# lyndonchan/wsss-analysis

Measured on AMD Instinct MI355X. Metric: images/sec CAM+CRF pseudo-labels, VOC2012 321x321, higher is better.
Workload: dtype f16x3; 1 GPU; resnet50 CAM + dense-CRF (M=21, 10 mean-field iters), 321x321, batch 32 images (=64 samples) per GPU, image-sharded; batch_images=32, num_classes=20, parallelism=image-sharded x1, no collective, steps_per_rank=243

## Files before the change

### include/wsscam.h

```cpp
#ifndef WSSCAM_H
#define WSSCAM_H

#include <stddef.h>
#include <stdint.h>

#ifdef __cplusplus
extern "C" {
#endif

#define WSC_VERSION 100

typedef enum wsc_status {
    WSC_OK = 0,
    WSC_ERR_INVALID = -1,
    WSC_ERR_NO_DEVICE = -2,
    WSC_ERR_HIP = -3,
    WSC_ERR_MISSING_KEY = -4,
    WSC_ERR_SHAPE = -5,
    WSC_ERR_NOMEM = -6,
    WSC_ERR_KEY_RANGE = -7,
    WSC_ERR_CAPACITY = -8,
    WSC_ERR_RANGE = -9
} wsc_status;

// ... 163 lines not shown

int wsc_hsn_gradcam_post(wsc_ctx *ctx, const float *cams_nhwc_dev, int B, int h, int w, int C, int S,
                         const float *gate_dev, float *out_dev, int out_channels, int out_first);
int wsc_hsn_voc_background(wsc_ctx *ctx, const float *Hbg_dev, int B, int Cb, int N, float *y_dev, int Ctot);
int wsc_hsn_class_mass(wsc_ctx *ctx, const float *maps_dev, int n_maps, int N, uint32_t *mass_dev);
int wsc_hsn_background(wsc_ctx *ctx, const uint8_t *rgb_dev, int B, int H, int W, int Ho, int Wo, double *bg_dev);
int wsc_cam_adp_modify(wsc_ctx *ctx, const float *cam_dev, int B, int n_sc, int C, int hw, const double *bg_dev, int mode,
                       const int32_t *use_host, int n_use, const int32_t *adipose_host, int n_adip, const int32_t *exc_host,
                       int n_exc, float *out_dev);
int wsc_hsn_cs_gradcam(wsc_ctx *ctx, const float *H_dev, int B, int C_all, int N, const double *bg_dev,
                       const int32_t *src_of_valid_host, int Cv, int bg_ind, int other_ind,
                       const int32_t *exception_inds_host, int n_exc, const int32_t *adipose_src_host, int n_adip,
                       float *cs_dev, float *y_dev, uint32_t *mass_dev);
int wsc_hsn_gather_unary(wsc_ctx *ctx, const float *maps_dev, const int64_t *chan_off_host, int n_chan, int N,
                         float *unary_dev);


int wsc_crf_create(wsc_ctx *ctx, const uint8_t *rgb_dev, int B, int H, int W, float g_sxy,
                   float bi_sxy, float bi_srgb, wsc_crf **out);
void wsc_crf_destroy(wsc_crf *crf);
int wsc_crf_lattice_sizes(wsc_ctx *ctx, const wsc_crf *crf, int32_t *v_gauss_host,
                          int32_t *v_bilat_host);
int wsc_crf_gaussian_on_chip(const wsc_crf *crf, int M);

int wsc_crf_inference(wsc_ctx *ctx, wsc_crf *crf, const float *unary_dev, int M, float g_compat,
                      float bi_compat, int n_iters, float *q_dev, int32_t *argmax_dev);
int wsc_crf_inference_pm(wsc_ctx *ctx, wsc_crf *crf, const float *unary_pm_dev, int M, float g_compat,
                         float bi_compat, int n_iters, float *q_dev, int32_t *argmax_dev);

int wsc_crf_v_create(wsc_ctx *ctx, const uint8_t *const *rgb_dev, const int32_t *hw_host , int B, float g_sxy,
                     float bi_sxy, float bi_srgb, wsc_crf_v **out);
void wsc_crf_v_destroy(wsc_crf_v *crf);
int wsc_crf_v_num_groups(const wsc_crf_v *crf);
int wsc_crf_v_inference(wsc_ctx *ctx, wsc_crf_v *crf, const float *const *unary_dev, const int32_t *M_host, float g_compat,
                        float bi_compat, int n_iters, float *const *q_dev, int32_t *const *argmax_dev);

#ifdef __cplusplus
}
#endif
#endif
```

### wsss-analysis_amd/csrc/crf.hip

```cpp
#include "common.h"

#include <atomic>
#include <cmath>
#include <cstring>
#include <memory>

namespace {

constexpr unsigned long long EMPTY_KEY = 0xFFFFFFFFFFFFFFFFull;
typedef float f32x2_t __attribute__((ext_vector_type(2)));

struct LatticeDev {
    int d = 0;
    int rep = 1;
    int rows = 0;
    int32_t *offset = nullptr;
    float *bary = nullptr;
    float *norm = nullptr;
    int2 *nbr = nullptr;
    int32_t *tslot_start = nullptr;
    int2 *slot_desc = nullptr;
    float *tent_w = nullptr;
    uint8_t *tent_p = nullptr;
    int32_t *row_slot_start = nullptr;
    int n_tiles = 0, n_slots = 0;
    bool sorted_dest = false;
    long long n_pix = 0;
    int M_cur = 0;
// ... 1628 lines not shown
                uint2 en[3];
                f32x4_t in[3];
#pragma unroll
                for (int jj = 0; jj < 3; ++jj) en[jj] = le[min(i + jj, n - 1)];
#pragma unroll
                for (int jj = 0; jj < 3; ++jj) in[jj] = stage[en[jj].x + l];
#pragma unroll
                for (int jj = 0; jj < 3; ++jj) {
                    const float w = i + jj < n ? __uint_as_float(en[jj].y) : 0.f;
                    const f32x2_t w2 = {w, w}, lo = {in[jj][0], in[jj][1]}, hi = {in[jj][2], in[jj][3]};
                    a01 = __builtin_elementwise_fma(w2, lo, a01);
                    a23 = __builtin_elementwise_fma(w2, hi, a23);
                }
            }
            const f32x4_t acc = {a01[0], a01[1], a23[0], a23[1]};
            if (ok) part[(unsigned)d.y * (unsigned)LP + l] = acc;
        }
        __syncthreads();
    }
}

constexpr int REC_LDS_BYTES = 56;
static_assert(TILE_PIX * REC_LDS_BYTES <= (int)(sizeof(uint2) * GATHER_ENT + sizeof(int2) * GATHER_SB), "record stage");
template <bool SLICE, bool SPLAT, bool GF = false, int FG = 0>
__global__ __launch_bounds__(512) __attribute__((amdgpu_waves_per_eu(4))) void update_splat_kernel(UpdateArgs a) {
    constexpr bool DMA = GF || (!SLICE && SPLAT);
    static_assert(!GF || SLICE, "the GF updates slice");
    static_assert(FG == 0 || GF, "the in-kernel Gaussian message belongs to the GF updates");
    extern __shared__ f32x4_t stage[];
    const int LP = a.LP;
    const int gpw = 64 / LP;
    const int lane = threadIdx.x & 63;
    const int g = lane / LP;
    const int l = lane - g * LP;
    const bool act = g < gpw;
    const int seg0 = g * LP;
    const int nb = gridDim.x, bid = blockIdx.x;
    const int xcd = bid & 7, qq = nb >> 3, rr = nb & 7;
    const int lb = (xcd < rr ? xcd * (qq + 1) : rr * (qq + 1) + (xcd - rr) * qq) + (bid >> 3);
    const int k = lb / a.tg.tpi, j = lb - k * a.tg.tpi;
    const TileBox tb = tile_box(a.tg, j);
    const int np = tb.cw * tb.ch;
    const int N = a.tg.H * a.tg.W;
    const int ppt = (int)(blockDim.x >> 6) * gpw;
    const unsigned cw_magic = tile_div_magic(tb.cw);
    const size_t pix0 = (size_t)k * (size_t)N + (size_t)tb.y0 * (size_t)a.tg.W + (size_t)tb.x0;
    const unsigned LP16 = (unsigned)LP * 16u, l16 = (unsigned)l * 16u;
    constexpr unsigned REC_BYTES = GF ? 52u : 80u;
// ... 72 lines not shown
            o23 = f32x2_t{u[2], u[3]};
        } else {
            o01 = f32x2_t{-u[0], -u[1]};
            o23 = f32x2_t{-u[2], -u[3]};
        }
        if (SLICE) {
            if (!GF) {
#pragma unroll
                for (int r = 0; r < 3; ++r) {
                    const f32x2_t w2 = {w9[r], w9[r]}, lo = {g3[r][0], g3[r][1]}, hi = {g3[r][2], g3[r][3]};
                    o01 = __builtin_elementwise_fma(w2, lo, o01);
                    o23 = __builtin_elementwise_fma(w2, hi, o23);
                }
            }
#pragma unroll
            for (int r = 0; r < 6; ++r) {
                const f32x2_t w2 = {w9[3 + r], w9[3 + r]}, lo = {b6[r][0], b6[r][1]}, hi = {b6[r][2], b6[r][3]};
                o01 = __builtin_elementwise_fma(w2, lo, o01);
                o23 = __builtin_elementwise_fma(w2, hi, o23);
            }
        }
    };
    const int t_first = (int)(threadIdx.x >> 6) * gpw;
    constexpr int EN_G = (TILE_PIX * 3 + 255) / 256, EN_B = (TILE_PIX * 6 + 255) / 256;
    SplatRegs<EN_G> rg;
    if (SPLAT && FG == 0) splat_fetch<EN_G>(a.sg, a.sg.shared ? j : lb, (a.sg.shared ? 0ll : (long long)k * N) + tb.ebase, np, rg);
    int4 cnt = make_int4(0, 0, 0, 0);
    int2 ps[FG > 0 ? FG : 1];
    uint4 tn0 = make_uint4(0, 0, 0, 0);
    if (FG > 0) {
        cnt = a.gt_cnt[j];
        const unsigned lpm = (65536u + (unsigned)LP - 1u) / (unsigned)LP;
        const int2 *trow = a.gt_rows + (size_t)j * a.gt_stride;
#pragma unroll
        for (int it = 0; it < (FG > 0 ? FG : 1); ++it) {
            const int i = (int)threadIdx.x + it * GM_THREADS;
            ps[it] = make_int2(0, 0);
            if (i < a.gt_stride * LP) ps[it] = trow[((unsigned)i * lpm) >> 16];
        }
        if ((int)threadIdx.x < a.gt_stride) tn0 = a.gt_nbr[(size_t)j * a.gt_stride + threadIdx.x];
    }
    if (DMA) {
        const int wvu = __builtin_amdgcn_readfirstlane((int)(threadIdx.x >> 6)), nwv = (int)(blockDim.x >> 6);
        const unsigned lp_magic = (65536u + (unsigned)LP - 1u) / (unsigned)LP;
        const int nE = np * LP;
        for (int u0 = wvu * 64; u0 < nE; u0 += nwv * 64) {
            const unsigned u = min((unsigned)(u0 + lane), (unsigned)(nE - 1));
            const unsigned t = (u * lp_magic) >> 16, ll = u - t * (unsigned)LP;
            const unsigned ty = (t * cw_magic) >> 16, tx = t - __umul24(ty, (unsigned)tb.cw);
            const char *src = u_b + (__umul24(__umul24(ty, (unsigned)a.tg.W) + tx, LP16) + ll * 16u);
            __builtin_amdgcn_global_load_lds((const __attribute__((address_space(1))) void *)src,
                                             (__attribute__((address_space(3))) void *)(reinterpret_cast<char *>(stage) + u0 * 16), 16, 0, 0);
        }
        const int nR = SLICE ? np * 14 : 0;
        for (int d0 = wvu * 64; d0 < nR; d0 += nwv * 64) {
            const unsigned d = min((unsigned)(d0 + lane), (unsigned)(nR - 1));
            const unsigned t = (d * 4682u) >> 16;
            const unsigned kk = min(d - t * 14u, 12u);
            const unsigned ty = (t * cw_magic) >> 16, tx = t - __umul24(ty, (unsigned)tb.cw);
            const char *src = rec_b + (__umul24(__umul24(ty, (unsigned)a.tg.W) + tx, REC_BYTES) + kk * 4u);
            __builtin_amdgcn_global_load_lds((const __attribute__((address_space(1))) void *)src,
                                             (__attribute__((address_space(3))) void *)(const_cast<char *>(lrec) + d0 * 4), 4, 0, 0);
        }
        if (FG == 0) {
            asm volatile("s_waitcnt vmcnt(0)" ::: "memory");
            __syncthreads();
        }
    }
    if constexpr (FG > 0) {
        constexpr int NIT = FG, NPI = FG == 4 ? 3 : 4;
        f32x4_t *gl = reinterpret_cast<f32x4_t *>(reinterpret_cast<char *>(stage + TILE_PIX * LP) + SPLAT_TAB_BYTES);
        const int stride = a.gt_stride, tid = (int)threadIdx.x;
        unsigned *lnb = reinterpret_cast<unsigned *>(gl + (size_t)stride * (size_t)LP);
        const f32x4_t zero = {0.f, 0.f, 0.f, 0.f};
        const f32x4_t *partg = reinterpret_cast<const f32x4_t *>(a.part_g_in) + (a.sg.shared ? (size_t)k * a.sg.n_slots * LP : (size_t)0);
        const int nitems_all = stride * LP;
        const unsigned lp_magic = (65536u + (unsigned)LP - 1u) / (unsigned)LP;
        const uint4 *tn = a.gt_nbr + (size_t)j * stride;
        const unsigned gpix0 = (unsigned)tb.y0 * (unsigned)a.tg.W + (unsigned)tb.x0;
        {
            f32x4_t val[NIT];
#pragma unroll
            for (int it = 0; it < NIT; ++it) {
                const int i = tid + it * GM_THREADS;
                const unsigned v = ((unsigned)i * lp_magic) >> 16, ll = (unsigned)i - v * (unsigned)LP;
                val[it] = zero;
                if (ps[it].y > 0) val[it] = partg[(unsigned)ps[it].x * (unsigned)LP + ll];
            }
            if (tid < stride) reinterpret_cast<uint4 *>(lnb)[tid] = tn0;
            for (int v = tid + GM_THREADS; v < stride; v += GM_THREADS) reinterpret_cast<uint4 *>(lnb)[v] = tn[v];
            int maxc = 0;
#pragma unroll
            for (int it = 0; it < NIT; ++it) maxc = max(maxc, ps[it].y);
            constexpr int UN = NIT <= 4 ? 3 : 2;
            if (maxc > 1) {
                f32x4_t more[UN][NIT];
#pragma unroll
                for (int c = 1; c <= UN; ++c)
#pragma unroll
                    for (int it = 0; it < NIT; ++it) {
                        const int i = tid + it * GM_THREADS;
                        const unsigned v = ((unsigned)i * lp_magic) >> 16, ll = (unsigned)i - v * (unsigned)LP;
                        more[c - 1][it] = zero;
                        if (c < ps[it].y) more[c - 1][it] = partg[(unsigned)(ps[it].x + c) * (unsigned)LP + ll];
                    }
#pragma unroll
                for (int c = 1; c <= UN; ++c)
#pragma unroll
                    for (int it = 0; it < NIT; ++it)
                        if (c < ps[it].y) {
#pragma unroll
                            for (int q = 0; q < 4; ++q) val[it][q] += more[c - 1][it][q];
                        }
            }
            for (int c = UN + 1; c < maxc; ++c) {
                f32x4_t more[NIT];
#pragma unroll
                for (int it = 0; it < NIT; ++it) {
                    const int i = tid + it * GM_THREADS;
                    const unsigned v = ((unsigned)i * lp_magic) >> 16, ll = (unsigned)i - v * (unsigned)LP;
                    more[it] = zero;
                    if (c < ps[it].y) more[it] = partg[(unsigned)(ps[it].x + c) * (unsigned)LP + ll];
                }
#pragma unroll
                for (int it = 0; it < NIT; ++it)
                    if (c < ps[it].y) {
#pragma unroll
                        for (int q = 0; q < 4; ++q) val[it][q] += more[it][q];
                    }
            }
#pragma unroll
            for (int it = 0; it < NIT; ++it) {
                const int i = tid + it * GM_THREADS;
                if (i < nitems_all) gl[i] = val[it];
            }
        }
        asm volatile("s_waitcnt vmcnt(0)" ::: "memory");
        uint4 gpx[NPI];
#pragma unroll
        for (int it = 0; it < NPI; ++it) {
            const int i = tid + it * GM_THREADS;
            gpx[it] = make_uint4(0, 0, 0, 0);
            if (i < np * LP) {
                const unsigned t = ((unsigned)i * lp_magic) >> 16;
                const unsigned ty = (t * cw_magic) >> 16, tx = t - ty * (unsigned)tb.cw;
                gpx[it] = a.gt_pix[gpix0 + ty * (unsigned)a.tg.W + tx];
            }
        }
        __syncthreads();
#pragma unroll
        for (int axis = 0; axis < 3; ++axis) {
            const int nitems = (axis == 0 ? cnt.z : (axis == 1 ? cnt.y : cnt.x)) * LP;
            f32x4_t o[NIT];
#pragma unroll
            for (int it = 0; it < NIT; ++it) {
                const int i = tid + it * GM_THREADS;
                o[it] = zero;
                if (i < nitems) {
                    const unsigned v = ((unsigned)i * lp_magic) >> 16, ll = (unsigned)i - v * (unsigned)LP;
                    const unsigned w = lnb[v * 4 + axis];
                    const f32x4_t c = gl[i], x1 = gl[(w & 0xffffu) * (unsigned)LP + ll], x2 = gl[(w >> 16) * (unsigned)LP + ll];
#pragma unroll
                    for (int q = 0; q < 4; ++q) o[it][q] = c[q] + 0.5f * (x1[q] + x2[q]);
                }
            }
            __syncthreads();
#pragma unroll
            for (int it = 0; it < NIT; ++it) {
                const int i = tid + it * GM_THREADS;
                if (i < nitems) gl[i] = o[it];
            }
            __syncthreads();
        }
#pragma unroll
        for (int it = 0; it < NPI; ++it) {
            const int i = tid + it * GM_THREADS;
            if (i < np * LP) {
                const unsigned t = ((unsigned)i * lp_magic) >> 16, ll = (unsigned)i - t * (unsigned)LP;
                const uint4 gp = gpx[it];
                const f32x4_t uu = stage[i];
                f32x2_t o01 = {-uu[0], -uu[1]}, o23 = {-uu[2], -uu[3]};
                const float wr[3] = {__uint_as_float(gp.y) * cag, __uint_as_float(gp.z) * cag, __uint_as_float(gp.w) * cag};
#pragma unroll
                for (int r = 0; r < 3; ++r) {
                    const f32x4_t row = gl[((gp.x >> (10 * r)) & 1023u) * (unsigned)LP + ll];
                    const f32x2_t w2 = {wr[r], wr[r]}, lo = {row[0], row[1]}, hi = {row[2], row[3]};
                    o01 = __builtin_elementwise_fma(w2, lo, o01);
                    o23 = __builtin_elementwise_fma(w2, hi, o23);
                }
                stage[i] = f32x4_t{o01[0], o01[1], o23[0], o23[1]};
            }
        }
        if (SPLAT) splat_fetch<EN_G>(a.sg, a.sg.shared ? j : lb, (a.sg.shared ? 0ll : (long long)k * N) + tb.ebase, np, rg);
        __syncthreads();
    }
    auto emit = [&](int t0) {
        const int t = t0 + g;
        const bool ok = act && t < np;
        const unsigned p = pixel_of(t0);
        float e[4] = {e01[0], e01[1], e23[0], e23[1]};
        float mx = -3.0e38f;
#pragma unroll
        for (int kk = 0; kk < 4; ++kk) {
            e[kk] = (ok && 4 * l + kk < a.M) ? e[kk] : -3.0e38f;
            mx = fmaxf(mx, e[kk]);
        }
        for (int o = 4; o > 0; o >>= 1) {
            const float other = __shfl_down(mx, o, 64);
            if (l + o < LP) mx = fmaxf(mx, other);
        }
        mx = __shfl(mx, seg0, 64);
        float ex[4], sum = 0.f;
        const float mxl = mx * 1.44269504088896341f;
#pragma unroll
        for (int kk = 0; kk < 4; ++kk) {
            ex[kk] = __builtin_amdgcn_exp2f(__builtin_fmaf(e[kk], 1.44269504088896341f, -mxl));
            sum += ex[kk];
// ... 19 lines not shown
                    bi = 4 * l + kk;
                }
            for (int o = 4; o > 0; o >>= 1) {
                const float ov = __shfl_down(bv, o, 64);
                const int oi = __shfl_down(bi, o, 64);
                if (l + o < LP && ov > bv) {
                    bv = ov;
                    bi = oi;
                }
            }
            if (ok && l == 0) a.argmax[pix0 + p] = bi;
        }
    };
    {
        {
            const f32x4_t u0 = load_u(t_first);
            f32x4_t g3[3], b6[6];
            float w9[9];
            if (SLICE) {
                load_rec(t_first, rq);
                issue_rows(rq, g3, b6, w9);
            }
            unn = u0;
            if (t_first + ppt < np) {
                if (SLICE) load_rec(t_first + ppt, rq);
                unn = load_u(t_first + ppt);
            }
            fold(u0, g3, b6, w9, e01, e23);
        }
        for (int t0 = t_first; t0 < np; t0 += ppt) {
            const bool has_next = t0 + ppt < np;
            f32x4_t vgn[3], vbn[6];
            float wrn[9];
            const f32x4_t un1 = unn;
            if (SLICE && has_next) issue_rows(rq, vgn, vbn, wrn);
            if (t0 + 2 * ppt < np) {
                if (SLICE) load_rec(t0 + 2 * ppt, rq);
                unn = load_u(t0 + 2 * ppt);
            }
            emit(t0);
            if (has_next) fold(un1, vgn, vbn, wrn, e01, e23);
        }
    }
    if (SPLAT) {
        uint2 *lent = reinterpret_cast<uint2 *>(stage + TILE_PIX * LP);
        int2 *ldesc = reinterpret_cast<int2 *>(lent + GATHER_ENT);
        if (DMA) __syncthreads();
        splat_commit<EN_G>(a.sg, np, rg, lent, ldesc, LP);
        SplatRegs<EN_B> rb;
        splat_fetch<EN_B>(a.sb, a.sb.shared ? j : lb, (a.sb.shared ? 0ll : (long long)k * N) + tb.ebase, np, rb);
        __syncthreads();
        tile_gather(a.sg, rg.s_beg, rg.s_end, k, stage, lent, ldesc, LP, l, g, gpw, act);
        splat_commit<EN_B>(a.sb, np, rb, lent, ldesc, LP);
        __syncthreads();
        tile_gather(a.sb, rb.s_beg, rb.s_end, k, stage, lent, ldesc, LP, l, g, gpw, act);
    }
}

struct GaussMsgArgs {
    const int4 *gt_cnt;
    const int2 *gt_rows;
    const uint4 *gt_nbr;
    const uint4 *gt_pix;
    const float *part;
    const float *u;
    float *e;
    int gt_stride, n_slots, shared, LP, B;
    float cag;
    TileGeom tg;
// ... 634 lines not shown
    WSC_TRY(tmp.alloc(sizeof(float) * L.rows, &va));
    WSC_TRY(tmp.alloc(sizeof(float) * L.rows, &vb));
    WSC_TRY(tmp.alloc(sizeof(float) * (size_t)(L.n_slots + 1), &vp));
    splat_ones(ctx, L, make_geom(crf->H, crf->W), va, vp);
    float *res = blur_all1(ctx, L, va, vb);
    uint32_t *rec_b = nullptr;
    if (D == 5 && !shared && crf->lat[0].gt_rows && !crf->pix_rec_b) WSC_TRY(own.alloc(sizeof(uint32_t) * 13 * (size_t)npix, &rec_b));
    if (!shared && D == 5) {
        hipLaunchKernelGGL(slice_norm_tile_kernel, dim3((unsigned)L.n_tiles), dim3(256), 0, ctx->stream, L.offset, L.bary, dp1,
                           L.alpha, res, make_geom(crf->H, crf->W), L.norm, rec_b, L.tent_w, L.tent_p);
    } else {
        hipLaunchKernelGGL(slice_norm_kernel, dim3(grid1d(npix)), dim3(256), 0, ctx->stream, L.offset, L.bary, dp1,
                           L.alpha, res, npix, L.norm, rec_b);
        hipLaunchKernelGGL(tile_scale_entries_kernel, dim3((unsigned)L.n_tiles), dim3(256), 0, ctx->stream, L.norm, dp1,
                           make_geom(crf->H, crf->W), L.tent_w, L.tent_p);
    }
    WSC_HIP(hipGetLastError());
    if (rec_b) crf->pix_rec_b = rec_b;
    return WSC_OK;
}

size_t update_splat_lds(int LP) { return sizeof(f32x4_t) * TILE_PIX * LP + sizeof(uint2) * GATHER_ENT + sizeof(int2) * GATHER_SB; }
size_t gauss_msg_lds(int LP, int gt_stride) { return ((size_t)LP * sizeof(f32x4_t) + sizeof(uint4)) * (size_t)gt_stride; }
size_t update_fg_lds(int LP, int gt_stride) { return update_splat_lds(LP) + gauss_msg_lds(LP, gt_stride); }
bool update_gf_ok(const wsc_ctx *ctx, const LatticeDev &G, int LP) {
    if (!ctx->opt[WSC_OPT_CRF_GAUSS_ON_CHIP]) return false;
    if (!G.gt_rows || G.rep < 1 || G.gt_stride <= 0) return false;
    if ((long long)G.gt_stride * LP > 6ll * GM_THREADS || (long long)G.gt_stride * LP >= 8192) return false;
    return gauss_msg_lds(LP, G.gt_stride) <= 64 * 1024;
}
bool update_fg_ok(const wsc_ctx *ctx, const LatticeDev &G, int LP) {
    if (!ctx->opt[WSC_OPT_CRF_MSG_IN_UPDATE] || !update_gf_ok(ctx, G, LP)) return false;
    return update_fg_lds(LP, G.gt_stride) <= 80 * 1024;
}
bool gauss_msg_small(int gt_stride, int LP) { return (long long)gt_stride * LP <= 4ll * GM_THREADS && LP <= 6; }

int launch_gauss_msg(wsc_ctx *ctx, hipStream_t st, const GaussMsgArgs &g, double bytes) {
    WscKernelTimer timer(ctx, WSC_K_GAUSS_MSG, bytes);
    const auto kernel = gauss_msg_small(g.gt_stride, g.LP) ? gauss_msg_kernel<4, 3> : gauss_msg_kernel<6, 4>;
    hipLaunchKernelGGL(kernel, dim3((unsigned)(g.B * g.tg.tpi)), dim3(GM_THREADS), gauss_msg_lds(g.LP, g.gt_stride), st, g);
    WSC_HIP(hipGetLastError());
    return WSC_OK;
}

typedef void (*UpdateKernel)(UpdateArgs);
template <bool SLICE, bool GF, int FG>
UpdateKernel update_kernel(bool splat) { return splat ? update_splat_kernel<SLICE, true, GF, FG> : update_splat_kernel<SLICE, false, GF, FG>; }
struct UpdateVariant { UpdateKernel kernel; int threads; size_t lds; };
UpdateVariant update_variant(bool slice, bool splat, bool gf, bool fg, bool small, int LP, int gt_stride) {
    if (fg) return {small ? update_kernel<true, true, 4>(splat) : update_kernel<true, true, 6>(splat), GM_THREADS, update_fg_lds(LP, gt_stride)};
    if (slice && gf) return {update_kernel<true, true, 0>(splat), 256, update_splat_lds(LP)};
    return {slice ? update_kernel<true, false, 0>(splat) : update_kernel<false, false, 0>(splat), 256, splat ? update_splat_lds(LP) : 0};
}
int update_fg_lds_limit(wsc_ctx *ctx, int LP, int gt_stride) {
    if (update_fg_lds(LP, gt_stride) <= 48 * 1024) return WSC_OK;
    for (const bool small : {true, false})
        for (const bool splat : {true, false}) {
            const UpdateKernel k = update_variant(true, splat, true, true, small, LP, gt_stride).kernel;
            WSC_TRY(wsc_set_max_dynamic_lds(ctx, reinterpret_cast<const void *>(k), 96 * 1024));
        }
    return WSC_OK;
}
int launch_update(wsc_ctx *ctx, const UpdateArgs &a, bool slice, bool splat, bool gf, bool fg = false, double fg_bytes = 0.0) {
    const double npix = (double)a.B * a.tg.H * a.tg.W;
    const double by = npix * (2.0 * a.M * 4 + (slice ? (gf ? 6 * 8 + 1.0 * a.M * 4 : 9 * 8 + 2.0 * a.M * 4) : 0.0) +
                              (splat ? 9 * 8 + 2.0 * a.M * 4 : 0.0));
    WscKernelTimer timer(ctx, WSC_K_SLICE_UPDATE, by + (fg ? fg_bytes : 0.0));
    const UpdateVariant v = update_variant(slice, splat, gf, fg, gauss_msg_small(a.gt_stride, a.LP), a.LP, a.gt_stride);
    hipLaunchKernelGGL(v.kernel, dim3((unsigned)(a.B * a.tg.tpi)), dim3(v.threads), v.lds, ctx->stream, a);
    WSC_HIP(hipGetLastError());
    return WSC_OK;
}

SplatTab splat_tab(const LatticeDev &L, float *part) {
    return SplatTab{L.tslot_start, L.slot_desc, L.tent_w, L.tent_p, part, L.n_slots, L.rep > 1 ? 1 : 0, L.d + 1};
}
UpdateArgs update_args(const wsc_crf *crf, int M, float g_compat, float bi_compat, const float *u, float *partg, float *partb) {
    const LatticeDev &G = crf->lat[0], &Bl = crf->lat[1];
    UpdateArgs a;
    a.pix_rec = crf->pix_rec; a.pix_rec_b = crf->pix_rec_b; a.val_g = nullptr; a.val_b = nullptr;
    a.u = u; a.q = nullptr; a.argmax = nullptr;
    a.alpha_g = G.alpha; a.alpha_b = Bl.alpha; a.compat_g = g_compat; a.compat_b = bi_compat;
    a.M = M; a.LP = (M + 3) / 4; a.B = crf->B; a.tg = make_geom(crf->H, crf->W);
    a.g_pix = (unsigned)G.n_pix; a.g_rows = G.rep > 1 ? (unsigned)G.rows : 0u;
    a.sg = splat_tab(G, partg); a.sb = splat_tab(Bl, partb);
    a.gt_cnt = G.gt_cnt; a.gt_rows = G.gt_rows; a.gt_nbr = G.gt_nbr; a.gt_pix = G.gt_pix; a.gt_stride = G.gt_stride;
    a.part_g_in = nullptr;
    return a;
}
GaussMsgArgs gauss_msg_args(const wsc_crf *crf, int M, float g_compat, const float *part, const float *u, float *e) {
    const LatticeDev &G = crf->lat[0];
// ... 106 lines not shown
}

void wsc_crf_destroy(wsc_crf *crf) {
    if (!crf) return;
    if (crf->used_elsewhere && crf->use_ev) (void)hipStreamWaitEvent(crf->ctx->stream, crf->use_ev, 0);
    if (crf->gauss) crf->gauss->users -= 1;
    crf->blocks.release();
    if (crf->use_ev) (void)hipEventDestroy(crf->use_ev);
    delete crf;
}

int wsc_crf_lattice_sizes(wsc_ctx *ctx, const wsc_crf *crf, int32_t *v_gauss_host, int32_t *v_bilat_host) {
    WSC_CHECK(ctx && crf, WSC_ERR_INVALID, "wsc_crf_lattice_sizes: null argument");
    for (int b = 0; b < crf->B; ++b) {
        if (v_gauss_host) v_gauss_host[b] = crf->lat[0].v_per_image[b];
        if (v_bilat_host) v_bilat_host[b] = crf->lat[1].v_per_image[b];
    }
    return WSC_OK;
}

int wsc_crf_gaussian_on_chip(const wsc_crf *crf, int M) {
    if (!crf || M < 1 || M > 32) return 0;
    return update_gf_ok(crf->ctx, crf->lat[0], (M + 3) / 4) ? 1 : 0;
}

static int crf_inference_impl(wsc_ctx *ctx, wsc_crf *crf, const float *unary_dev, bool pixel_major, int M, float g_compat,
                              float bi_compat, int n_iters, float *q_dev, int32_t *argmax_dev);

int wsc_crf_inference(wsc_ctx *ctx, wsc_crf *crf, const float *unary_dev, int M, float g_compat, float bi_compat,
                      int n_iters, float *q_dev, int32_t *argmax_dev) {
    return crf_inference_impl(ctx, crf, unary_dev, false, M, g_compat, bi_compat, n_iters, q_dev, argmax_dev);
}

int wsc_crf_inference_pm(wsc_ctx *ctx, wsc_crf *crf, const float *unary_pm_dev, int M, float g_compat, float bi_compat,
                         int n_iters, float *q_dev, int32_t *argmax_dev) {
    return crf_inference_impl(ctx, crf, unary_pm_dev, true, M, g_compat, bi_compat, n_iters, q_dev, argmax_dev);
}

static int crf_inference_impl(wsc_ctx *ctx, wsc_crf *crf, const float *unary_dev, bool pixel_major, int M, float g_compat,
                              float bi_compat, int n_iters, float *q_dev, int32_t *argmax_dev) {
    WSC_CHECK(ctx && crf && unary_dev, WSC_ERR_INVALID, "wsc_crf_inference: null argument");
    WSC_CHECK(M >= 1 && M <= 32, WSC_ERR_INVALID, "wsc_crf_inference: M=%d outside [1,32]", M);
    WSC_CHECK(n_iters >= 0, WSC_ERR_INVALID, "wsc_crf_inference: n_iters=%d", n_iters);
    WSC_HIP(hipSetDevice(ctx->device));
    const int B = crf->B, N = crf->N;
    const long long npix = (long long)B * N;
// ... 21 lines not shown
    float *partg = (float *)p; p += pg;
    float *partg2 = (float *)p; p += pg;
    float *partb = (float *)p; p += pb;

    crf->lat[0].M_cur = M;
    crf->lat[1].M_cur = M;
    if (n_iters > 0) WSC_TRY(blur_lds_prepare(ctx, crf->lat[1], M));
    const dim3 tgrid((N + TP - 1) / TP, B);
    if (!pixel_major) {
        WscKernelTimer timer(ctx, WSC_K_CRF_MISC, (double)npix * M * 12);
        hipLaunchKernelGGL(init_q_kernel, tgrid, dim3(TP), 2 * (size_t)M * (TP + 1) * sizeof(float), ctx->stream,
                           unary_dev, M, Mp, N, u, n_iters == 0 ? q : (float *)nullptr);
    } else {
        u = const_cast<float *>(unary_dev);
    }
    const bool lds_blur = Bl.bl_ok && Bl.img_row && ctx->opt[WSC_OPT_CRF_BLUR_ON_CHIP];
    const bool no_fork = lds_blur || ctx->profiling;
    if (!no_fork && !ctx->aux_stream) {
        WSC_HIP(hipStreamCreateWithFlags(&ctx->aux_stream, hipStreamNonBlocking));
        WSC_HIP(hipEventCreateWithFlags(&ctx->fork_ev, hipEventDisableTiming));
        WSC_HIP(hipEventCreateWithFlags(&ctx->aux_done_ev, hipEventDisableTiming));
    }
    const bool gf = update_gf_ok(ctx, G, LP);
    const bool fg = gf && update_fg_ok(ctx, G, LP) && update_fg_lds_limit(ctx, LP, G.gt_stride) == WSC_OK;
    if (n_iters > 0) WSC_TRY(gf ? crf_bilateral_records(crf, ctx->stream) : crf_full_records(crf, ctx->stream));
    UpdateArgs a = update_args(crf, M, g_compat, bi_compat, u, partg, partb);
    const GaussMsgArgs gm = gauss_msg_args(crf, M, g_compat, partg, u, q);
    const double gf_bytes = 2.0 * 3.0 * (double)(G.rows - 1) * G.rep * M * 4 + (double)npix * (3 * 8 + 1.0 * M * 4);
    if (n_iters == 0 && pixel_major) {
        a.q = q;
        WSC_TRY(launch_update(ctx, a, false, false, false));
    }
    for (int it = 0; it <= n_iters && n_iters > 0; ++it) {
        const bool last = it == n_iters;
        const bool labels_only = last && q_dev == nullptr && argmax_dev != nullptr;
        a.q = last && !labels_only ? q : nullptr;
        a.argmax = labels_only ? argmax_dev : nullptr;
        a.u = (gf && !fg && it > 0) ? q : u;
        if (fg) {
            a.part_g_in = (it & 1) ? partg : partg2;
            a.sg.part = (it & 1) ? partg2 : partg;
        }
        WSC_TRY(launch_update(ctx, a, it > 0, !last, gf, fg && it > 0, gf_bytes));
        if (last) break;
        const bool fork = !no_fork;
        hipStream_t main_stream = ctx->stream;
        if (fork) {
// ... 148 lines not shown
```

### wsss-analysis_amd/wsscam/_lib.py

```python
import ctypes
import os
import re
import threading

import numpy as np

_HERE = os.path.dirname(os.path.abspath(__file__))
LIB_PATH = os.path.join(_HERE, "libwsscam.so")
HEADER_PATH = os.path.normpath(os.path.join(_HERE, "..", "..", "include", "wsscam.h"))

WSC_OK = 0
WSC_ERR_INVALID = -1
WSC_ERR_NO_DEVICE = -2
WSC_ERR_HIP = -3
WSC_ERR_MISSING_KEY = -4
WSC_ERR_SHAPE = -5
WSC_ERR_NOMEM = -6
WSC_ERR_KEY_RANGE = -7
WSC_ERR_CAPACITY = -8
WSC_ERR_RANGE = -9

ARCH_RESNET50_CAM = 0
ARCH_VGG16_CAM = 1
ARCH_M7_CAM = 2
# ... 82 lines not shown
    "wsc_unary_from_maps": (_i, [_vp, _vp, _i, _i, _i, _f, _vp]),
    "wsc_cam_unary": (_i, [_vp, _vp, _i, _i, _i, _i, _i, _i, _f, _vp]),
    "wsc_cam_unary_pm": (_i, [_vp, _vp, _i, _i, _i, _i, _i, _i, _f, _vp]),
    "wsc_cam_sum_scales": (_i, [_vp, _vp, _i, _i, ctypes.c_longlong, _vp]),
    "wsc_cam_eval_confusion_nn": (_i, [_vp, _vp, _i, _vp, _vp, _vp, _vp, _vp, _vp, _i, _i, _vp, _vp]),
    "wsc_label_confusion_nn": (_i, [_vp, _vp, _i, _vp, _vp, _vp, _vp, _i, _i, _vp, _vp]),
    "wsc_sem_seg_finish": (_i, [_vp, _vp, _i, _vp, _vp, _vp, _vp, _vp, _vp, _i, _f, _vp]),
    "wsc_bilinear_resize": (_i, [_vp, _vp, _i, _i, _i, _vp, _i, _i]),
    "wsc_msf_input_u8": (_i, [_vp, _vp, _i, _vp, _vp, _i, _vp, _vp, _i, _i, _vp]),
    "wsc_resize_u8": (_i, [_vp, _vp, _i, _vp, _vp, _i, _i, _vp]),
    "wsc_label_unary_from_cam": (_i, [_vp, _vp, _i, _i, _i, _f, _f, _vp, _vp]),
    "wsc_ir_label_combine": (_i, [_vp, _vp, _vp, _vp, _i, _i, _i, _vp]),
    "wsc_hsn_gradcam_post": (_i, [_vp, _vp, _i, _i, _i, _i, _i, _vp, _vp, _i, _i]),
    "wsc_hsn_voc_background": (_i, [_vp, _vp, _i, _i, _i, _vp, _i]),
    "wsc_hsn_class_mass": (_i, [_vp, _vp, _i, _i, _vp]),
    "wsc_hsn_background": (_i, [_vp, _vp, _i, _i, _i, _i, _i, _vp]),
    "wsc_cam_adp_modify": (_i, [_vp, _vp, _i, _i, _i, _i, _vp, _i, _vp, _i, _vp, _i, _vp, _i, _vp]),
    "wsc_hsn_cs_gradcam": (_i, [_vp, _vp, _i, _i, _i, _vp, _vp, _i, _i, _i, _vp, _i, _vp, _i, _vp, _vp, _vp]),
    "wsc_hsn_gather_unary": (_i, [_vp, _vp, _vp, _i, _i, _vp]),
    "wsc_crf_create": (_i, [_vp, _vp, _i, _i, _i, _f, _f, _f, ctypes.POINTER(_vp)]),
    "wsc_crf_destroy": (None, [_vp]),
    "wsc_crf_lattice_sizes": (_i, [_vp, _vp, _vp, _vp]),
    "wsc_crf_gaussian_on_chip": (_i, [_vp, _i]),
    "wsc_crf_inference": (_i, [_vp, _vp, _vp, _i, _f, _f, _i, _vp, _vp]),
    "wsc_crf_inference_pm": (_i, [_vp, _vp, _vp, _i, _f, _f, _i, _vp, _vp]),
    "wsc_crf_v_create": (_i, [_vp, _vp, _vp, _i, _f, _f, _f, ctypes.POINTER(_vp)]),
    "wsc_crf_v_destroy": (None, [_vp]),
    "wsc_crf_v_num_groups": (_i, [_vp]),
    "wsc_crf_v_inference": (_i, [_vp, _vp, _vp, _vp, _f, _f, _i, _vp, _vp]),
}


def header_symbols():
    with open(HEADER_PATH) as fh:
        text = fh.read()
    text = re.sub(r"/\*.*?\*/", "", text, flags=re.S)
    return sorted(set(re.findall(r"\b(wsc_[a-z0-9_]+)\s*\(", text)))


def load():
    global _lib
    if _lib is not None:
        return _lib
    if not os.path.exists(LIB_PATH):
        raise WscError(WSC_ERR_NO_DEVICE,
                       "libwsscam.so not built at %s -- run `python __graft_entry__.py` (there is no "
# ... 474 lines not shown
                                      ctypes.byref(h)))
        self.h = h

    def close(self):
        if getattr(self, "h", None) and self.ctx.h:
            self.ctx._lib.wsc_crf_destroy(self.h)
        self.h = None

    def __del__(self):
        try:
            self.close()
        except Exception:
            pass

    def lattice_sizes(self):
        vg = np.zeros(self.B, dtype=np.int32)
        vb = np.zeros(self.B, dtype=np.int32)
        check(self.ctx._lib.wsc_crf_lattice_sizes(self.ctx.h, self.h, vg.ctypes.data, vb.ctypes.data))
        return vg, vb

    def gaussian_on_chip(self, M):
        return bool(self.ctx._lib.wsc_crf_gaussian_on_chip(self.h, int(M)))

    def inference(self, unary_dev, M, g_compat, bi_compat, n_iters, q_dev=None, argmax_dev=None, ctx=None, pixel_major=False):
        run = ctx or self.ctx
        fn = self.ctx._lib.wsc_crf_inference_pm if pixel_major else self.ctx._lib.wsc_crf_inference
        check(fn(run.h, self.h, _ptr(unary_dev), M, float(g_compat), float(bi_compat), int(n_iters), _ptr(q_dev),
                 _ptr(argmax_dev)))


def _ptr_array(ptrs):
    arr = (ctypes.c_void_p * len(ptrs))()
    for i, p in enumerate(ptrs):
        arr[i] = None if p is None else (p.ptr if hasattr(p, "ptr") else int(p))
    return arr


class CrfV:

    def __init__(self, ctx, rgb_ptrs, sizes, g_sxy, bi_sxy, bi_srgb):
        self.ctx = ctx
        self.B = len(rgb_ptrs)
        self.sizes = [(int(h), int(w)) for h, w in sizes]
        assert len(self.sizes) == self.B
        hw = np.ascontiguousarray(self.sizes, dtype=np.int32).reshape(self.B, 2)
        arr = _ptr_array(rgb_ptrs)
# ... 132 lines not shown
```

Before: 2657 images/s.

## Process fused Gaussian message in column chunks to shrink LDS and raise occupancy

The fused in-update Gaussian blur now walks the lattice in chunks of CG=2 channel-columns instead of holding all LP columns in LDS at once. It prefetches the next chunk's partial sums while blurring the current one, and packs neighbour indices into 10-bit fields. Unary and record loads are deferred on this path, and the waves-per-EU hint goes up for the smaller variant. The aim is a much smaller LDS footprint so more blocks fit per CU, at the cost of more barriers and repeated axis passes per chunk. Eligibility is now decided by an occupancy query, cached per kernel, requiring at least 2 blocks per CU, and a diagnostic API exposes the chosen form.

```diff
diff --git a/include/wsscam.h b/include/wsscam.h
--- a/include/wsscam.h
+++ b/include/wsscam.h
@@ -209,6 +209,7 @@
 int wsc_crf_lattice_sizes(wsc_ctx *ctx, const wsc_crf *crf, int32_t *v_gauss_host,
                           int32_t *v_bilat_host);
 int wsc_crf_gaussian_on_chip(const wsc_crf *crf, int M);
+int wsc_crf_update_form(const wsc_crf *crf, int M, int32_t *threads, int32_t *lds_bytes, int32_t *blocks_per_cu);
 
 int wsc_crf_inference(wsc_ctx *ctx, wsc_crf *crf, const float *unary_dev, int M, float g_compat,
                       float bi_compat, int n_iters, float *q_dev, int32_t *argmax_dev);
diff --git a/wsss-analysis_amd/csrc/crf.hip b/wsss-analysis_amd/csrc/crf.hip
--- a/wsss-analysis_amd/csrc/crf.hip
+++ b/wsss-analysis_amd/csrc/crf.hip
@@ -3,7 +3,10 @@
 #include <atomic>
 #include <cmath>
 #include <cstring>
+#include <map>
 #include <memory>
+#include <mutex>
+#include <tuple>
 
 namespace {
 
@@ -1678,8 +1681,12 @@
 
 constexpr int REC_LDS_BYTES = 56;
 static_assert(TILE_PIX * REC_LDS_BYTES <= (int)(sizeof(uint2) * GATHER_ENT + sizeof(int2) * GATHER_SB), "record stage");
+constexpr int CG = 2;
+__device__ __forceinline__ uint2 pack_nbr(const uint4 &w) {
+    return make_uint2((w.x & 0xffffu) | ((w.y & 0xffffu) << 10) | ((w.z & 0xffffu) << 20), (w.x >> 16) | ((w.y >> 16) << 10) | ((w.z >> 16) << 20));
+}
 template <bool SLICE, bool SPLAT, bool GF = false, int FG = 0>
-__global__ __launch_bounds__(512) __attribute__((amdgpu_waves_per_eu(4))) void update_splat_kernel(UpdateArgs a) {
+__global__ __launch_bounds__(512) __attribute__((amdgpu_waves_per_eu(FG == 2 ? 6 : 4))) void update_splat_kernel(UpdateArgs a) {
     constexpr bool DMA = GF || (!SLICE && SPLAT);
     static_assert(!GF || SLICE, "the GF updates slice");
     static_assert(FG == 0 || GF, "the in-kernel Gaussian message belongs to the GF updates");
@@ -1798,7 +1805,9 @@
         }
     };
     const int t_first = (int)(threadIdx.x >> 6) * gpw;
-    constexpr int EN_G = (TILE_PIX * 3 + 255) / 256, EN_B = (TILE_PIX * 6 + 255) / 256;
+    constexpr bool LATE = FG > 0;
+    constexpr int BT = FG > 0 ? GM_THREADS : 256;
+    constexpr int EN_G = (TILE_PIX * 3 + BT - 1) / BT, EN_B = (TILE_PIX * 6 + BT - 1) / BT;
     SplatRegs<EN_G> rg;
     if (SPLAT && FG == 0) splat_fetch<EN_G>(a.sg, a.sg.shared ? j : lb, (a.sg.shared ? 0ll : (long long)k * N) + tb.ebase, np, rg);
     int4 cnt = make_int4(0, 0, 0, 0);
@@ -1806,13 +1815,12 @@
     uint4 tn0 = make_uint4(0, 0, 0, 0);
     if (FG > 0) {
         cnt = a.gt_cnt[j];
-        const unsigned lpm = (65536u + (unsigned)LP - 1u) / (unsigned)LP;
         const int2 *trow = a.gt_rows + (size_t)j * a.gt_stride;
 #pragma unroll
         for (int it = 0; it < (FG > 0 ? FG : 1); ++it) {
-            const int i = (int)threadIdx.x + it * GM_THREADS;
+            const int v = ((int)threadIdx.x + it * GM_THREADS) / CG;
             ps[it] = make_int2(0, 0);
-            if (i < a.gt_stride * LP) ps[it] = trow[((unsigned)i * lpm) >> 16];
+            if (v < a.gt_stride) ps[it] = trow[v];
         }
         if ((int)threadIdx.x < a.gt_stride) tn0 = a.gt_nbr[(size_t)j * a.gt_stride + threadIdx.x];
     }
@@ -1844,65 +1852,68 @@
         }
     }
     if constexpr (FG > 0) {
-        constexpr int NIT = FG, NPI = FG == 4 ? 3 : 4;
+        constexpr int NIT = FG;
+        static_assert(GM_THREADS == TILE_PIX * CG && GM_THREADS % CG == 0, "one slice item per thread");
         f32x4_t *gl = reinterpret_cast<f32x4_t *>(reinterpret_cast<char *>(stage + TILE_PIX * LP) + SPLAT_TAB_BYTES);
         const int stride = a.gt_stride, tid = (int)threadIdx.x;
-        unsigned *lnb = reinterpret_cast<unsigned *>(gl + (size_t)stride * (size_t)LP);
+        uint2 *lnb = reinterpret_cast<uint2 *>(gl + (size_t)stride * CG);
         const f32x4_t zero = {0.f, 0.f, 0.f, 0.f};
         const f32x4_t *partg = reinterpret_cast<const f32x4_t *>(a.part_g_in) + (a.sg.shared ? (size_t)k * a.sg.n_slots * LP : (size_t)0);
-        const int nitems_all = stride * LP;
-        const unsigned lp_magic = (65536u + (unsigned)LP - 1u) / (unsigned)LP;
+        const int nitems_all = stride * CG;
         const uint4 *tn = a.gt_nbr + (size_t)j * stride;
-        const unsigned gpix0 = (unsigned)tb.y0 * (unsigned)a.tg.W + (unsigned)tb.x0;
-        {
-            f32x4_t val[NIT];
+        const unsigned ll = (unsigned)tid % CG, pt = (unsigned)tid / CG;
+        if (tid < stride) lnb[tid] = pack_nbr(tn0);
+        for (int v = tid + GM_THREADS; v < stride; v += GM_THREADS) lnb[v] = pack_nbr(tn[v]);
+        int maxc = 0;
+#pragma unroll
+        for (int it = 0; it < NIT; ++it) maxc = max(maxc, ps[it].y);
+        uint4 gpx = make_uint4(0, 0, 0, 0);
+        constexpr int UN = 2;
+        f32x4_t val[NIT], more[UN][NIT];
+        auto request = [&](int c0) {
+            const unsigned col = (unsigned)c0 + ll;
+            const bool colok = col < (unsigned)LP;
 #pragma unroll
             for (int it = 0; it < NIT; ++it) {
-                const int i = tid + it * GM_THREADS;
-                const unsigned v = ((unsigned)i * lp_magic) >> 16, ll = (unsigned)i - v * (unsigned)LP;
                 val[it] = zero;
-                if (ps[it].y > 0) val[it] = partg[(unsigned)ps[it].x * (unsigned)LP + ll];
-            }
-            if (tid < stride) reinterpret_cast<uint4 *>(lnb)[tid] = tn0;
-            for (int v = tid + GM_THREADS; v < stride; v += GM_THREADS) reinterpret_cast<uint4 *>(lnb)[v] = tn[v];
-            int maxc = 0;
-#pragma unroll
-            for (int it = 0; it < NIT; ++it) maxc = max(maxc, ps[it].y);
-            constexpr int UN = NIT <= 4 ? 3 : 2;
+                if (colok && ps[it].y > 0) val[it] = partg[(unsigned)ps[it].x * (unsigned)LP + col];
+            }
             if (maxc > 1) {
-                f32x4_t more[UN][NIT];
 #pragma unroll
                 for (int c = 1; c <= UN; ++c)
 #pragma unroll
                     for (int it = 0; it < NIT; ++it) {
-                        const int i = tid + it * GM_THREADS;
-                        const unsigned v = ((unsigned)i * lp_magic) >> 16, ll = (unsigned)i - v * (unsigned)LP;
                         more[c - 1][it] = zero;
-                        if (c < ps[it].y) more[c - 1][it] = partg[(unsigned)(ps[it].x + c) * (unsigned)LP + ll];
+                        if (colok && c < ps[it].y) more[c - 1][it] = partg[(unsigned)(ps[it].x + c) * (unsigned)LP + col];
                     }
+            }
+        };
+        request(0);
+        for (int c0 = 0; c0 < LP; c0 += CG) {
+            const unsigned col = (unsigned)c0 + ll;
+            const bool colok = col < (unsigned)LP;
+            if (maxc > 1) {
 #pragma unroll
                 for (int c = 1; c <= UN; ++c)
 #pragma unroll
                     for (int it = 0; it < NIT; ++it)
-                        if (c < ps[it].y) {
+                        if (colok && c < ps[it].y) {
 #pragma unroll
                             for (int q = 0; q < 4; ++q) val[it][q] += more[c - 1][it][q];
                         }
             }
             for (int c = UN + 1; c < maxc; ++c) {
-                f32x4_t more[NIT];
+                f32x4_t mo[NIT];
 #pragma unroll
                 for (int it = 0; it < NIT; ++it) {
-                    const int i = tid + it * GM_THREADS;
-                    const unsigned v = ((unsigned)i * lp_magic) >> 16, ll = (unsigned)i - v * (unsigned)LP;
-                    more[it] = zero;
-                    if (c < ps[it].y) more[it] = partg[(unsigned)(ps[it].x + c) * (unsigned)LP + ll];
+                    mo[it] = zero;
+                    if (colok && c < ps[it].y) mo[it] = partg[(unsigned)(ps[it].x + c) * (unsigned)LP + col];
                 }
 #pragma unroll
                 for (int it = 0; it < NIT; ++it)
-                    if (c < ps[it].y) {
-#pragma unroll
-                        for (int q = 0; q < 4; ++q) val[it][q] += more[it][q];
+                    if (colok && c < ps[it].y) {
+#pragma unroll
+                        for (int q = 0; q < 4; ++q) val[it][q] += mo[it][q];
                     }
             }
 #pragma unroll
@@ -1910,65 +1921,55 @@
                 const int i = tid + it * GM_THREADS;
                 if (i < nitems_all) gl[i] = val[it];
             }
-        }
-        asm volatile("s_waitcnt vmcnt(0)" ::: "memory");
-        uint4 gpx[NPI];
-#pragma unroll
-        for (int it = 0; it < NPI; ++it) {
-            const int i = tid + it * GM_THREADS;
-            gpx[it] = make_uint4(0, 0, 0, 0);
-            if (i < np * LP) {
-                const unsigned t = ((unsigned)i * lp_magic) >> 16;
-                const unsigned ty = (t * cw_magic) >> 16, tx = t - ty * (unsigned)tb.cw;
-                gpx[it] = a.gt_pix[gpix0 + ty * (unsigned)a.tg.W + tx];
-            }
-        }
-        __syncthreads();
-#pragma unroll
-        for (int axis = 0; axis < 3; ++axis) {
-            const int nitems = (axis == 0 ? cnt.z : (axis == 1 ? cnt.y : cnt.x)) * LP;
-            f32x4_t o[NIT];
-#pragma unroll
-            for (int it = 0; it < NIT; ++it) {
-                const int i = tid + it * GM_THREADS;
-                o[it] = zero;
-                if (i < nitems) {
-                    const unsigned v = ((unsigned)i * lp_magic) >> 16, ll = (unsigned)i - v * (unsigned)LP;
-                    const unsigned w = lnb[v * 4 + axis];
-                    const f32x4_t c = gl[i], x1 = gl[(w & 0xffffu) * (unsigned)LP + ll], x2 = gl[(w >> 16) * (unsigned)LP + ll];
-#pragma unroll
-                    for (int q = 0; q < 4; ++q) o[it][q] = c[q] + 0.5f * (x1[q] + x2[q]);
+            if (c0 == 0) {
+                asm volatile("s_waitcnt vmcnt(0)" ::: "memory");
+                if ((int)pt < np) {
+                    const unsigned ty = (pt * cw_magic) >> 16, tx = pt - ty * (unsigned)tb.cw;
+                    gpx = a.gt_pix[(unsigned)tb.y0 * (unsigned)a.tg.W + (unsigned)tb.x0 + ty * (unsigned)a.tg.W + tx];
                 }
             }
+            if (c0 + CG < LP) request(c0 + CG);
             __syncthreads();
 #pragma unroll
-            for (int it = 0; it < NIT; ++it) {
-                const int i = tid + it * GM_THREADS;
-                if (i < nitems) gl[i] = o[it];
-            }
-            __syncthreads();
-        }
-#pragma unroll
-        for (int it = 0; it < NPI; ++it) {
-            const int i = tid + it * GM_THREADS;
-            if (i < np * LP) {
-                const unsigned t = ((unsigned)i * lp_magic) >> 16, ll = (unsigned)i - t * (unsigned)LP;
-                const uint4 gp = gpx[it];
-                const f32x4_t uu = stage[i];
+            for (int axis = 0; axis < 3; ++axis) {
+                const int nitems = (axis == 0 ? cnt.z : (axis == 1 ? cnt.y : cnt.x)) * CG;
+                f32x4_t o[NIT];
+#pragma unroll
+                for (int it = 0; it < NIT; ++it) {
+                    const int i = tid + it * GM_THREADS;
+                    o[it] = zero;
+                    if (colok && i < nitems) {
+                        const uint2 w = lnb[(unsigned)i / CG];
+                        const unsigned n1 = (w.x >> (10 * axis)) & 1023u, n2 = (w.y >> (10 * axis)) & 1023u;
+                        const f32x4_t c = gl[i], x1 = gl[n1 * CG + ll], x2 = gl[n2 * CG + ll];
+#pragma unroll
+                        for (int q = 0; q < 4; ++q) o[it][q] = c[q] + 0.5f * (x1[q] + x2[q]);
+                    }
+                }
+                __syncthreads();
+#pragma unroll
+                for (int it = 0; it < NIT; ++it) {
+                    const int i = tid + it * GM_THREADS;
+                    if (colok && i < nitems) gl[i] = o[it];
+                }
+                __syncthreads();
+            }
+            if (colok && (int)pt < np) {
+                const unsigned si = pt * (unsigned)LP + col;
+                const f32x4_t uu = stage[si];
                 f32x2_t o01 = {-uu[0], -uu[1]}, o23 = {-uu[2], -uu[3]};
-                const float wr[3] = {__uint_as_float(gp.y) * cag, __uint_as_float(gp.z) * cag, __uint_as_float(gp.w) * cag};
+                const float wr[3] = {__uint_as_float(gpx.y) * cag, __uint_as_float(gpx.z) * cag, __uint_as_float(gpx.w) * cag};
 #pragma unroll
                 for (int r = 0; r < 3; ++r) {
-                    const f32x4_t row = gl[((gp.x >> (10 * r)) & 1023u) * (unsigned)LP + ll];
+                    const f32x4_t row = gl[((gpx.x >> (10 * r)) & 1023u) * CG + ll];
                     const f32x2_t w2 = {wr[r], wr[r]}, lo = {row[0], row[1]}, hi = {row[2], row[3]};
                     o01 = __builtin_elementwise_fma(w2, lo, o01);
                     o23 = __builtin_elementwise_fma(w2, hi, o23);
                 }
-                stage[i] = f32x4_t{o01[0], o01[1], o23[0], o23[1]};
-            }
-        }
-        if (SPLAT) splat_fetch<EN_G>(a.sg, a.sg.shared ? j : lb, (a.sg.shared ? 0ll : (long long)k * N) + tb.ebase, np, rg);
-        __syncthreads();
+                stage[si] = f32x4_t{o01[0], o01[1], o23[0], o23[1]};
+            }
+            __syncthreads();
+        }
     }
     auto emit = [&](int t0) {
         const int t = t0 + g;
@@ -2034,7 +2035,7 @@
                 issue_rows(rq, g3, b6, w9);
             }
             unn = u0;
-            if (t_first + ppt < np) {
+            if (!LATE && t_first + ppt < np) {
                 if (SLICE) load_rec(t_first + ppt, rq);
                 unn = load_u(t_first + ppt);
             }
@@ -2045,18 +2046,22 @@
             f32x4_t vgn[3], vbn[6];
             float wrn[9];
             const f32x4_t un1 = unn;
-            if (SLICE && has_next) issue_rows(rq, vgn, vbn, wrn);
-            if (t0 + 2 * ppt < np) {
+            if (SLICE && has_next) {
+                if (LATE) load_rec(t0 + ppt, rq);
+                issue_rows(rq, vgn, vbn, wrn);
+            }
+            if (!LATE && t0 + 2 * ppt < np) {
                 if (SLICE) load_rec(t0 + 2 * ppt, rq);
                 unn = load_u(t0 + 2 * ppt);
             }
             emit(t0);
-            if (has_next) fold(un1, vgn, vbn, wrn, e01, e23);
+            if (has_next) fold(LATE ? load_u(t0 + ppt) : un1, vgn, vbn, wrn, e01, e23);
         }
     }
     if (SPLAT) {
         uint2 *lent = reinterpret_cast<uint2 *>(stage + TILE_PIX * LP);
         int2 *ldesc = reinterpret_cast<int2 *>(lent + GATHER_ENT);
+        if (FG > 0) splat_fetch<EN_G>(a.sg, a.sg.shared ? j : lb, (a.sg.shared ? 0ll : (long long)k * N) + tb.ebase, np, rg);
         if (DMA) __syncthreads();
         splat_commit<EN_G>(a.sg, np, rg, lent, ldesc, LP);
         SplatRegs<EN_B> rb;
@@ -2737,17 +2742,15 @@
 
 size_t update_splat_lds(int LP) { return sizeof(f32x4_t) * TILE_PIX * LP + sizeof(uint2) * GATHER_ENT + sizeof(int2) * GATHER_SB; }
 size_t gauss_msg_lds(int LP, int gt_stride) { return ((size_t)LP * sizeof(f32x4_t) + sizeof(uint4)) * (size_t)gt_stride; }
-size_t update_fg_lds(int LP, int gt_stride) { return update_splat_lds(LP) + gauss_msg_lds(LP, gt_stride); }
+size_t update_fg_lds(int LP, int gt_stride) { return update_splat_lds(LP) + (CG * sizeof(f32x4_t) + sizeof(uint2)) * (size_t)gt_stride; }
 bool update_gf_ok(const wsc_ctx *ctx, const LatticeDev &G, int LP) {
     if (!ctx->opt[WSC_OPT_CRF_GAUSS_ON_CHIP]) return false;
     if (!G.gt_rows || G.rep < 1 || G.gt_stride <= 0) return false;
     if ((long long)G.gt_stride * LP > 6ll * GM_THREADS || (long long)G.gt_stride * LP >= 8192) return false;
     return gauss_msg_lds(LP, G.gt_stride) <= 64 * 1024;
 }
-bool update_fg_ok(const wsc_ctx *ctx, const LatticeDev &G, int LP) {
-    if (!ctx->opt[WSC_OPT_CRF_MSG_IN_UPDATE] || !update_gf_ok(ctx, G, LP)) return false;
-    return update_fg_lds(LP, G.gt_stride) <= 80 * 1024;
-}
+int update_fg_items(int gt_stride) { return gt_stride * CG <= 2 * GM_THREADS ? 2 : 4; }
+static_assert((GT_MAX_LOCAL + 1) * CG <= 4 * GM_THREADS, "FG = 4 covers the largest tile vertex set");
 bool gauss_msg_small(int gt_stride, int LP) { return (long long)gt_stride * LP <= 4ll * GM_THREADS && LP <= 6; }
 
 int launch_gauss_msg(wsc_ctx *ctx, hipStream_t st, const GaussMsgArgs &g, double bytes) {
@@ -2762,26 +2765,40 @@
 template <bool SLICE, bool GF, int FG>
 UpdateKernel update_kernel(bool splat) { return splat ? update_splat_kernel<SLICE, true, GF, FG> : update_splat_kernel<SLICE, false, GF, FG>; }
 struct UpdateVariant { UpdateKernel kernel; int threads; size_t lds; };
-UpdateVariant update_variant(bool slice, bool splat, bool gf, bool fg, bool small, int LP, int gt_stride) {
-    if (fg) return {small ? update_kernel<true, true, 4>(splat) : update_kernel<true, true, 6>(splat), GM_THREADS, update_fg_lds(LP, gt_stride)};
+UpdateVariant update_variant(bool slice, bool splat, bool gf, bool fg, int LP, int gt_stride) {
+    if (fg) return {update_fg_items(gt_stride) == 2 ? update_kernel<true, true, 2>(splat) : update_kernel<true, true, 4>(splat), GM_THREADS, update_fg_lds(LP, gt_stride)};
     if (slice && gf) return {update_kernel<true, true, 0>(splat), 256, update_splat_lds(LP)};
     return {slice ? update_kernel<true, false, 0>(splat) : update_kernel<false, false, 0>(splat), 256, splat ? update_splat_lds(LP) : 0};
 }
-int update_fg_lds_limit(wsc_ctx *ctx, int LP, int gt_stride) {
-    if (update_fg_lds(LP, gt_stride) <= 48 * 1024) return WSC_OK;
-    for (const bool small : {true, false})
-        for (const bool splat : {true, false}) {
-            const UpdateKernel k = update_variant(true, splat, true, true, small, LP, gt_stride).kernel;
-            WSC_TRY(wsc_set_max_dynamic_lds(ctx, reinterpret_cast<const void *>(k), 96 * 1024));
-        }
-    return WSC_OK;
+int update_blocks_per_cu(wsc_ctx *ctx, const UpdateVariant &v) {
+    static std::mutex mu;
+    static std::map<std::tuple<const void *, int, size_t>, int> known;
+    const void *fn = reinterpret_cast<const void *>(v.kernel);
+    std::lock_guard<std::mutex> lock(mu);
+    const auto key = std::make_tuple(fn, ctx->device, v.lds);
+    const auto hit = known.find(key);
+    if (hit != known.end()) return hit->second;
+    int lds_cu = 0, blocks = 0;
+    if (hipDeviceGetAttribute(&lds_cu, hipDeviceAttributeMaxSharedMemoryPerMultiprocessor, ctx->device) != hipSuccess) lds_cu = 0;
+    if (v.lds <= (size_t)lds_cu && (v.lds <= 48 * 1024 || wsc_set_max_dynamic_lds(ctx, fn, lds_cu) == WSC_OK)) {
+        if (hipOccupancyMaxActiveBlocksPerMultiprocessor(&blocks, fn, v.threads, v.lds) != hipSuccess) blocks = 0;
+    }
+    (void)hipGetLastError();
+    known[key] = blocks;
+    return blocks;
+}
+bool update_fg_ok(wsc_ctx *ctx, const LatticeDev &G, int LP) {
+    if (!ctx->opt[WSC_OPT_CRF_MSG_IN_UPDATE] || !update_gf_ok(ctx, G, LP)) return false;
+    for (const bool splat : {true, false})
+        if (update_blocks_per_cu(ctx, update_variant(true, splat, true, true, LP, G.gt_stride)) < 2) return false;
+    return true;
 }
 int launch_update(wsc_ctx *ctx, const UpdateArgs &a, bool slice, bool splat, bool gf, bool fg = false, double fg_bytes = 0.0) {
     const double npix = (double)a.B * a.tg.H * a.tg.W;
     const double by = npix * (2.0 * a.M * 4 + (slice ? (gf ? 6 * 8 + 1.0 * a.M * 4 : 9 * 8 + 2.0 * a.M * 4) : 0.0) +
                               (splat ? 9 * 8 + 2.0 * a.M * 4 : 0.0));
     WscKernelTimer timer(ctx, WSC_K_SLICE_UPDATE, by + (fg ? fg_bytes : 0.0));
-    const UpdateVariant v = update_variant(slice, splat, gf, fg, gauss_msg_small(a.gt_stride, a.LP), a.LP, a.gt_stride);
+    const UpdateVariant v = update_variant(slice, splat, gf, fg, a.LP, a.gt_stride);
     hipLaunchKernelGGL(v.kernel, dim3((unsigned)(a.B * a.tg.tpi)), dim3(v.threads), v.lds, ctx->stream, a);
     WSC_HIP(hipGetLastError());
     return WSC_OK;
@@ -2934,6 +2951,20 @@
 int wsc_crf_gaussian_on_chip(const wsc_crf *crf, int M) {
     if (!crf || M < 1 || M > 32) return 0;
     return update_gf_ok(crf->ctx, crf->lat[0], (M + 3) / 4) ? 1 : 0;
+}
+
+int wsc_crf_update_form(const wsc_crf *crf, int M, int32_t *threads, int32_t *lds_bytes, int32_t *blocks_per_cu) {
+    WSC_CHECK(crf && M >= 1 && M <= 32, WSC_ERR_INVALID, "wsc_crf_update_form: null crf or M=%d outside [1,32]", M);
+    WSC_HIP(hipSetDevice(crf->ctx->device));
+    const int LP = (M + 3) / 4;
+    const LatticeDev &G = crf->lat[0];
+    const bool gf = update_gf_ok(crf->ctx, G, LP);
+    const bool fg = gf && update_fg_ok(crf->ctx, G, LP);
+    const UpdateVariant v = update_variant(true, true, gf, fg, LP, G.gt_stride);
+    if (threads) *threads = v.threads;
+    if (lds_bytes) *lds_bytes = (int32_t)v.lds;
+    if (blocks_per_cu) *blocks_per_cu = update_blocks_per_cu(crf->ctx, v);
+    return fg ? 1 : 0;
 }
 
 static int crf_inference_impl(wsc_ctx *ctx, wsc_crf *crf, const float *unary_dev, bool pixel_major, int M, float g_compat,
@@ -3001,7 +3032,7 @@
         WSC_HIP(hipEventCreateWithFlags(&ctx->aux_done_ev, hipEventDisableTiming));
     }
     const bool gf = update_gf_ok(ctx, G, LP);
-    const bool fg = gf && update_fg_ok(ctx, G, LP) && update_fg_lds_limit(ctx, LP, G.gt_stride) == WSC_OK;
+    const bool fg = gf && update_fg_ok(ctx, G, LP);
     if (n_iters > 0) WSC_TRY(gf ? crf_bilateral_records(crf, ctx->stream) : crf_full_records(crf, ctx->stream));
     UpdateArgs a = update_args(crf, M, g_compat, bi_compat, u, partg, partb);
     const GaussMsgArgs gm = gauss_msg_args(crf, M, g_compat, partg, u, q);
diff --git a/wsss-analysis_amd/wsscam/_lib.py b/wsss-analysis_amd/wsscam/_lib.py
--- a/wsss-analysis_amd/wsscam/_lib.py
+++ b/wsss-analysis_amd/wsscam/_lib.py
@@ -128,6 +128,7 @@
     "wsc_crf_destroy": (None, [_vp]),
     "wsc_crf_lattice_sizes": (_i, [_vp, _vp, _vp, _vp]),
     "wsc_crf_gaussian_on_chip": (_i, [_vp, _i]),
+    "wsc_crf_update_form": (_i, [_vp, _i, _vp, _vp, _vp]),
     "wsc_crf_inference": (_i, [_vp, _vp, _vp, _i, _f, _f, _i, _vp, _vp]),
     "wsc_crf_inference_pm": (_i, [_vp, _vp, _vp, _i, _f, _f, _i, _vp, _vp]),
     "wsc_crf_v_create": (_i, [_vp, _vp, _vp, _i, _f, _f, _f, ctypes.POINTER(_vp)]),
@@ -648,6 +649,13 @@
     def gaussian_on_chip(self, M):
         return bool(self.ctx._lib.wsc_crf_gaussian_on_chip(self.h, int(M)))
 
+    def update_form(self, M):
+        v = np.zeros(3, dtype=np.int32)
+        st = self.ctx._lib.wsc_crf_update_form(self.h, int(M), v.ctypes.data, v.ctypes.data + 4, v.ctypes.data + 8)
+        if st < 0:
+            check(st)
+        return bool(st), int(v[0]), int(v[1]), int(v[2])
+
     def inference(self, unary_dev, M, g_compat, bi_compat, n_iters, q_dev=None, argmax_dev=None, ctx=None, pixel_major=False):
         run = ctx or self.ctx
         fn = self.ctx._lib.wsc_crf_inference_pm if pixel_major else self.ctx._lib.wsc_crf_inference
```

After: 2596 images/s. 2.3% lower.
